# BUTSpeechFIT/DiariZen

Hardware: AMD Instinct MI355X
Metric: audio-seconds/s (RTF) for wavlm-large-s80 pipeline, 16 kHz mono (higher is better)
Workload: dtype f32 (operands split into 2 fp16 terms with exact power-of-two scaling = 22 significant bits, 3 fp16 MFMA products, fp32 accumulate: the error-corrected '3xFP16/3xTF32' scheme; kernels without an fp16 variant use the 3-term bf16 split)

## Files before the change

diarizen_amd/_lib.py:

```python
from __future__ import annotations

import ctypes as C
import os
from pathlib import Path

DZN_MAX_CONV = 8
DZN_MAX_LAYERS = 32
DZN_MAX_HEADS = 16

DZN_PREC_F32 = 0
DZN_PREC_BF16 = 1
DZN_PREC_F32_SPLIT = 2
DZN_PREC_F32_H2 = 3
DZN_PREC_F16 = 4

DZN_ACT_NONE, DZN_ACT_GELU, DZN_ACT_SWISH, DZN_ACT_RELU = 0, 1, 2, 3

DZN_F32, DZN_F64, DZN_I64 = 0, 1, 2

ERRORS = {0: "ok", -1: "invalid argument", -2: "out of memory", -3: "HIP runtime error",
          -4: "bad call order", -5: "missing state_dict key"}


class DznError(RuntimeError):
# ... 15 lines not shown
        ("embed_dim", C.c_int32),
        ("total_heads", C.c_int32),
        ("n_layers", C.c_int32),
        ("layer_norm_first", C.c_int32),
        ("pos_conv_kernel", C.c_int32),
        ("pos_conv_groups", C.c_int32),
        ("num_buckets", C.c_int32),
        ("max_distance", C.c_int32),
        ("use_attention", C.c_int32 * DZN_MAX_LAYERS),
        ("n_heads", C.c_int32 * DZN_MAX_LAYERS),
        ("head_idx", (C.c_int32 * DZN_MAX_HEADS) * DZN_MAX_LAYERS),
        ("use_ffn", C.c_int32 * DZN_MAX_LAYERS),
        ("ffn_dim", C.c_int32 * DZN_MAX_LAYERS),
        ("attention_in", C.c_int32),
        ("ffn_hidden", C.c_int32),
        ("conf_heads", C.c_int32),
        ("conf_layers", C.c_int32),
        ("conf_kernel", C.c_int32),
        ("n_classes", C.c_int32),
        ("max_speakers_per_chunk", C.c_int32),
        ("max_speakers_per_frame", C.c_int32),
        ("has_embedding", C.c_int32),
        ("embed_out_dim", C.c_int32),
        ("num_mel_bins", C.c_int32),
        ("reserved", C.c_int32 * 16),
    ]


class DznGemmDesc(C.Structure):
    _fields_ = [
        ("A", C.c_void_p), ("W", C.c_void_p), ("W16", C.c_void_p), ("C", C.c_void_p),
        ("bias", C.c_void_p), ("R", C.c_void_p), ("WS", C.c_void_p),
        ("a_rowoff", C.c_void_p), ("c_rowoff", C.c_void_p),
        ("M", C.c_int32), ("N", C.c_int32), ("K", C.c_int32),
        ("lda", C.c_int64), ("kc", C.c_int32), ("ldk", C.c_int64), ("ldw", C.c_int32),
        ("ldc", C.c_int64), ("ldws", C.c_int64),
        ("act", C.c_int32), ("alpha", C.c_float), ("post_relu", C.c_int32),
        ("ws_w", C.c_float), ("ws_init", C.c_int32),
        ("nz", C.c_int32), ("zdiv", C.c_int32),
        ("a_z0", C.c_int64), ("a_z1", C.c_int64), ("w_z0", C.c_int64), ("w_z1", C.c_int64),
        ("c_z0", C.c_int64), ("c_z1", C.c_int64), ("b_z0", C.c_int64), ("b_z1", C.c_int64),
        ("precision", C.c_int32),
        ("alg_flops", C.c_double),
        ("W3", C.c_void_p),
        ("a_split3", C.c_int32), ("a_plane", C.c_int64),
        ("ln_stats", C.c_void_p), ("ln_colsum", C.c_void_p),
        ("W2h", C.c_void_p), ("col_scale", C.c_void_p), ("a_amax", C.c_void_p), ("c_amax", C.c_void_p),
        ("amax_unit", C.c_int32),
        ("stat_partial", C.c_void_p), ("stat_final", C.c_void_p), ("stat_C", C.c_int32), ("stat_eps", C.c_float),
        ("z_count", C.c_void_p), ("z_list", C.c_void_p),
        ("Wmx", C.c_void_p), ("col_scale_mx", C.c_void_p),
        ("amax_count", C.c_int32),
        ("kv_planes", C.c_void_p), ("kv_plane_stride", C.c_int64), ("kv_scale", C.c_void_p), ("kv_ld", C.c_int32),
        ("kv_col0", C.c_int32),
        ("A2", C.c_void_p), ("a2_rowoff", C.c_void_p), ("a2_amax", C.c_void_p), ("a2_z0", C.c_int64),
        ("k1", C.c_int32), ("k2", C.c_int32),
    ]


class DznProfEntry(C.Structure):
    _fields_ = [("name", C.c_char * 64), ("launches", C.c_int64), ("ms", C.c_double),
                ("flops", C.c_double), ("bytes", C.c_double)]


def lib_path() -> Path:
    env = os.environ.get("DZN_HIP_LIB")
    if env:
        return Path(env)
    return Path(__file__).resolve().parent / "lib" / "libdzn_hip.so"


_LIB = None


def load() -> C.CDLL:
    global _LIB
    if _LIB is not None:
        return _LIB
    p = lib_path()
    if not p.exists():
        raise DznError(
            f"{p} not found: build the HIP extension first (python -m diarizen_amd.build). "
            "diarizen_amd has no CPU fallback.")
    try:
        import torch
    except Exception:
        pass
    lib = C.CDLL(str(p))
    vp, i32, i64, f32 = C.c_void_p, C.c_int32, C.c_int64, C.c_float

    def sig(name, res, args):
        fn = getattr(lib, name)
        fn.restype = res
        fn.argtypes = args

    sig("dzn_create", i32, [C.POINTER(DznConfig), C.POINTER(vp)])
    sig("dzn_load_tensor", i32, [vp, C.c_char_p, vp, C.POINTER(i64), i32, i32])
    sig("dzn_finalize_weights", i32, [vp])
    sig("dzn_num_frames", i32, [vp, i32])
    sig("dzn_segment_forward", i32, [vp, vp, i32, i32, vp, vp, vp])
    sig("dzn_segment_forward_soft", i32, [vp, vp, i32, i32, vp, vp, vp, vp])
    sig("dzn_embed_forward", i32, [vp, vp, vp, i32, i32, i32, i32, vp, vp])
    sig("dzn_prepare_masks", i32, [vp, vp, i32, i32, i32, i32, i32, vp, vp, vp])
    sig("dzn_speaker_count", i32, [vp, i32, i32, i32, vp, i32, vp, vp, vp])
    sig("dzn_cluster_activations", i32, [vp, vp, i32, i32, i32, vp, i32, i32, vp, vp])
    sig("dzn_detect", i32, [vp, i32, i32, i32, vp, vp, i32, i32, f32, f32, vp, vp, vp])
    sig("dzn_speaker_scores", i32, [vp, vp, i32, i32, i32, vp, vp, vp, i32, i32, vp, vp])
    sig("dzn_debug_fetch", i32, [vp, C.c_char_p, vp, i64, C.POINTER(i64)])
    sig("dzn_embed_skip_stats", i32, [vp, C.POINTER(i64), C.POINTER(i64)])
    sig("dzn_num_ignored", i32, [vp])
    sig("dzn_workspace_bytes", i64, [vp])
    sig("dzn_last_error", C.c_char_p, [vp])
    sig("dzn_destroy", i32, [vp])
    sig("dzn_version", C.c_char_p, [])
    sig("dzn_profile_enable", i32, [i32])
    sig("dzn_profile_collect", i32, [C.POINTER(DznProfEntry), i32, C.POINTER(i32)])
    sig("dzn_profile_reserve", i32, [i32])
    sig("dzn_op_relpos_bucket", i32, [i32, i32, i32])
    sig("dzn_linkage_centroid", i32, [vp, i32, i32, vp, i32])
    sig("dzn_cdist_cosine", i32, [vp, i32, i32, vp, i32, vp, i32])
    sig("dzn_host_workspace_release", i32, [i32])
    sig("dzn_host_workspace_bytes", i64, [i32])
    sig("dzn_vbx_create", i32, [vp, vp, vp, i32, i32, i32, i32, C.POINTER(C.c_void_p)])
    sig("dzn_vbx_stats", i32, [vp, vp])
    sig("dzn_vbx_estep", i32, [vp, vp, vp, vp, C.c_double, C.POINTER(C.c_double)])
    sig("dzn_vbx_gamma", i32, [vp, vp])
    sig("dzn_vbx_destroy", i32, [vp])
    sig("dzn_op_gemm", i32, [C.POINTER(DznGemmDesc), vp])
    sig("dzn_op_split_weights", i32, [vp, i64, i32, i64, vp, vp])
    sig("dzn_op_split_weights_h2", i32, [vp, i64, i32, i64, vp, vp, vp])
    sig("dzn_op_split_weights_mx", i32, [vp, i64, i32, i64, vp, vp, vp])
    sig("dzn_op_set_gemm_mx_cfg", i32, [C.c_char_p])
    sig("dzn_checked_status", i32, [vp, i32])
    sig("dzn_flac_info", i32, [vp, C.c_size_t, vp, vp, vp, vp, vp])
    sig("dzn_flac_decode", i32, [vp, C.c_size_t, vp, i64, vp])
    sig("dzn_op_set_gemm_cfg", i32, [C.c_char_p])
    sig("dzn_op_amax", i32, [vp, i64, vp, vp])
    sig("dzn_op_split_rows", i32, [vp, vp, i64, i64, i32, vp])
    sig("dzn_op_conv3x3_c32", i32, [vp, vp, vp, vp, vp, i32, i32, i32, i32, i32, vp])
    sig("dzn_op_resblock_ws", i32, [vp, vp, vp, vp, vp, vp, vp, vp, vp, f32, f32, i32, i32, i32, i32, vp])
    sig("dzn_op_resblock32_fused", i32, [vp, vp, vp, vp, vp, vp, vp, vp, vp, f32, f32, i32, i32, i32, vp])
    sig("dzn_op_set_resblock_np", i32, [i32])
    sig("dzn_op_set_attention_noskip", i32, [i32])
    sig("dzn_op_conv3x3_c32_h2", i32, [vp, vp, vp, vp, vp, vp, vp, vp, i32, i32, i32, i32, i32, vp])
    sig("dzn_op_layernorm", i32, [vp, i64, vp, i64, vp, vp, i64, i32, i32, f32, i32, vp])
    sig("dzn_op_gate", i32, [vp, i64, vp, vp, vp, vp, i64, i32, vp])
    sig("dzn_op_row_stats", i32, [vp, i64, i64, i32, f32, vp, vp])
    sig("dzn_op_gate_stats", i32, [vp, i64, vp, vp, vp, vp, vp, vp, vp, i64, i32, f32, vp])
    sig("dzn_op_attention_h2", i32, [vp, vp, vp, vp, vp, i32, i32, i32, i32, i32, i32, f32, vp, vp])
    sig("dzn_op_set_attention_qb", i32, [i32])
    sig("dzn_op_set_attention_prefetch", i32, [i32])
    sig("dzn_op_attention_planes", i32, [vp, vp, vp, vp, vp, i32, i32, i32, i32, i32, i32, f32, vp, vp, vp, vp])
    sig("dzn_op_attention", i32, [vp, vp, vp, vp, vp, i32, i32, i32, i32, i32, i32, f32, i32, vp])
    _LIB = lib
    return lib


EXPORTED = [
    "dzn_create", "dzn_load_tensor", "dzn_finalize_weights", "dzn_num_frames",
    "dzn_segment_forward", "dzn_segment_forward_soft", "dzn_embed_forward", "dzn_prepare_masks", "dzn_speaker_count", "dzn_cluster_activations", "dzn_detect", "dzn_speaker_scores", "dzn_debug_fetch", "dzn_embed_skip_stats", "dzn_num_ignored",
    "dzn_workspace_bytes", "dzn_last_error", "dzn_destroy", "dzn_version", "dzn_linkage_centroid", "dzn_cdist_cosine", "dzn_host_workspace_release",
    "dzn_host_workspace_bytes",
    "dzn_flac_info", "dzn_flac_decode", "dzn_vbx_create", "dzn_vbx_stats", "dzn_vbx_estep", "dzn_vbx_gamma", "dzn_vbx_destroy",
    "dzn_op_gemm", "dzn_op_split_weights", "dzn_op_split_weights_h2", "dzn_op_split_weights_mx", "dzn_op_set_gemm_mx_cfg", "dzn_checked_status", "dzn_op_set_gemm_cfg", "dzn_op_amax", "dzn_op_conv3x3_c32", "dzn_op_conv3x3_c32_h2", "dzn_op_resblock32_fused", "dzn_op_resblock_ws", "dzn_op_set_resblock_np", "dzn_op_set_attention_noskip", "dzn_op_split_rows", "dzn_op_layernorm", "dzn_op_row_stats", "dzn_op_gate", "dzn_op_gate_stats", "dzn_op_attention", "dzn_op_attention_h2", "dzn_op_attention_planes", "dzn_op_set_attention_qb", "dzn_op_set_attention_prefetch",
    "dzn_profile_enable", "dzn_profile_collect", "dzn_profile_reserve", "dzn_op_relpos_bucket",
]


def profile_enable(on: bool) -> None:
    check(load().dzn_profile_enable(int(on)), None, "dzn_profile_enable")


def profile_reserve(n_events: int) -> None:
    check(load().dzn_profile_reserve(int(n_events)), None, "dzn_profile_reserve")


def profile_collect() -> list:
    lib = load()
    arr = (DznProfEntry * 512)()
    n = C.c_int32(0)
    check(lib.dzn_profile_collect(arr, 512, C.byref(n)), None, "dzn_profile_collect")
    return [dict(name=arr[i].name.decode(), launches=arr[i].launches, ms=arr[i].ms,
                 flops=arr[i].flops, bytes=arr[i].bytes) for i in range(min(n.value, 512))]


def check(rc: int, handle=None, what: str = "") -> None:
    if rc == 0:
        return
    msg = ERRORS.get(rc, f"error {rc}")
    try:
        detail = load().dzn_last_error(handle)
        if detail:
            msg += ": " + detail.decode(errors="replace")
    except Exception:
        pass
    if rc == -2:
        raise MemoryError(f"{what}: {msg}")
    raise DznError(f"{what}: {msg}")
```

diarizen_amd/csrc/conformer.hip:

```cpp
#include "common.h"

namespace {

constexpr int DW_TT = 32;

template <int KS>
__global__ __launch_bounds__(256) void glu_dwconv_kernel(const float* __restrict__ u, int64_t ldu,
                                                         const float* __restrict__ w,
                                                         const float* __restrict__ bias,
                                                         float* __restrict__ out, int64_t ldo, int L,
                                                         int A) {
  constexpr int PAD = (KS - 1) / 2;
  constexpr int NIN = DW_TT + KS - 1;
  const int b = blockIdx.y;
  const int t0 = blockIdx.x * DW_TT;
  for (int c = threadIdx.x; c < A; c += blockDim.x) {
    float wr[KS];
#pragma unroll
    for (int j = 0; j < KS; ++j) wr[j] = w[c * KS + j];
    const float bc = bias[c];
    float in[NIN];
#pragma unroll
    for (int i = 0; i < NIN; ++i) {
      const int t = t0 - PAD + i;
      float v = 0.f;
      if (t >= 0 && t < L) {
        const float* up = u + ((int64_t)b * L + t) * ldu;
        v = up[c] * sigmoidf_(up[A + c]);
      }
      in[i] = v;
    }
#pragma unroll
    for (int t = 0; t < DW_TT; ++t) {
      if (t0 + t < L) {
        float a = 0.f;
#pragma unroll
        for (int j = 0; j < KS; ++j) a = fmaf(in[t + j], wr[j], a);
        a += bc;
        out[((int64_t)b * L + t0 + t) * ldo + c] = swishf_(a);
      }
    }
  }
}

__global__ __launch_bounds__(256) void classify_kernel(const float* __restrict__ z, int64_t ldz,
                                                       const float* __restrict__ W,
                                                       const float* __restrict__ bias,
                                                       const uint8_t* __restrict__ mapping,
                                                       int64_t rows, int A, int NC, int S,
                                                       float* __restrict__ logp,
                                                       uint8_t* __restrict__ multilabel,
                                                       float* __restrict__ soft) {
  const int lane = threadIdx.x & 63, wave = threadIdx.x >> 6;
  const int64_t row = (int64_t)blockIdx.x * 4 + wave;
  if (row >= rows) return;
  const float* zp = z + row * ldz;
  float logit[16];
#pragma unroll
  for (int c = 0; c < 16; ++c) logit[c] = 0.f;
  for (int i = lane; i < A; i += 64) {
    const float v = zp[i];
#pragma unroll
    for (int c = 0; c < 16; ++c)
      if (c < NC) logit[c] = fmaf(v, W[c * A + i], logit[c]);
  }
  float mx = -INFINITY;
  int arg = 0;
#pragma unroll
  for (int c = 0; c < 16; ++c) {
    if (c < NC) {
      logit[c] = wave_sum(logit[c]) + bias[c];
      if (logit[c] > mx) { mx = logit[c]; arg = c; }
    }
  }
  float se = 0.f;
#pragma unroll
  for (int c = 0; c < 16; ++c)
    if (c < NC) se += expf(logit[c] - mx);
  const float lse = mx + logf(se);
  if (logp) {
#pragma unroll
    for (int c = 0; c < 16; ++c)
      if (c < NC && lane == c) logp[row * NC + c] = logit[c] - lse;
  }
  if (multilabel && lane < S) multilabel[row * S + lane] = mapping[arg * S + lane];
  if (soft && lane < S) {
    float p = 0.f;
#pragma unroll
    for (int c = 0; c < 16; ++c)
      if (c < NC && mapping[c * S + lane]) p += expf(logit[c] - lse);
    soft[row * S + lane] = p;
  }
}

}

int launch_glu_dwconv(const float* u, int64_t ldu, const float* w, const float* bias, float* out,
                      int64_t ldo, int B, int L, int A, int ks, hipStream_t st) {
  ProfScope prof_scope_(st, "glu_dwconv", 0.0, (double)B * L * A * 12.0);
  dim3 grid((L + DW_TT - 1) / DW_TT, B);
  const int threads = A >= 256 ? 256 : (A >= 128 ? 128 : 64);
#define DZN_DW(KSV) \
  hipLaunchKernelGGL((glu_dwconv_kernel<KSV>), grid, dim3(threads), 0, st, u, ldu, w, bias, out, ldo, L, A)
  if (ks == 31) DZN_DW(31);
  else if (ks == 7) DZN_DW(7);
  else if (ks == 15) DZN_DW(15);
  else return DZN_E_INVALID;
#undef DZN_DW
  return hipGetLastError() == hipSuccess ? DZN_OK : DZN_E_HIP;
}

int launch_classify(const float* z, int64_t ldz, const float* W, const float* bias,
                    const uint8_t* mapping, int64_t rows, int A, int NC, int S, float* logp,
                    uint8_t* multilabel, float* soft, hipStream_t st) {
  ProfScope prof_scope_(st, "classify", 2.0 * (double)rows * A * NC,
                        (double)rows * (A * 4.0 + NC * 4.0 + S + (soft ? S * 4.0 : 0.0)));
  if (NC > 16 || S > 64) return DZN_E_INVALID;
  hipLaunchKernelGGL(classify_kernel, dim3((unsigned)cdiv64(rows, 4)), dim3(256), 0, st, z, ldz, W,
                     bias, mapping, rows, A, NC, S, logp, multilabel, soft);
  return hipGetLastError() == hipSuccess ? DZN_OK : DZN_E_HIP;
}
```

diarizen_amd/csrc/embed.hip:

```cpp

#include "common.h"

namespace {

__global__ __launch_bounds__(256) void frame_prep_kernel(const float* __restrict__ wave, int N,
                                                         int T, int flen, int fshift, int Kp,
                                                         const float* __restrict__ window,
                                                         float preemph, float* __restrict__ frames) {
  const int lane = threadIdx.x & 63, wv = threadIdx.x >> 6;
  const int b = blockIdx.y;
  const int t = blockIdx.x * 4 + wv;
  if (t >= T) return;
  const float* xp = wave + (int64_t)b * N + (int64_t)t * fshift;
  float v[8];
  float s = 0.f;
#pragma unroll
  for (int i = 0; i < 8; ++i) {
    const int idx = lane + 64 * i;
    v[i] = idx < flen ? xp[idx] * 32768.0f : 0.f;
    s += v[i];
  }
  const float mean = wave_sum(s) / (float)flen;
  float* op = frames + ((int64_t)b * T + t) * Kp;
  float pv[8];
#pragma unroll
  for (int i = 0; i < 8; ++i) {
    float prev = __shfl_up(v[i], 1, 64);
    const float prev_reg = __shfl(v[i > 0 ? i - 1 : 0], 63, 64);
    if (lane == 0) prev = i > 0 ? prev_reg : v[0];
    pv[i] = prev;
  }
#pragma unroll
  for (int i = 0; i < 8; ++i) {
    const int idx = lane + 64 * i;
    if (idx < flen) {
      const float cur = v[i] - mean;
      const float prev = pv[i] - mean;
      op[idx] = (cur - preemph * prev) * window[idx];
    } else if (idx < Kp) {
      op[idx] = 0.f;
    }
  }
}

__global__ __launch_bounds__(256) void power_kernel(const float* __restrict__ spec, int64_t rows,
                                                    int nb, float* __restrict__ pw) {
  const int64_t n = rows * nb;
  for (int64_t i = (int64_t)blockIdx.x * 256 + threadIdx.x; i < n; i += (int64_t)gridDim.x * 256) {
    const int64_t r = i / nb;
    const int f = (int)(i - r * nb);
    const float re = spec[r * 2 * nb + f], im = spec[r * 2 * nb + nb + f];
    const float a = sqrtf(re * re + im * im);
    pw[i] = a * a;
  }
}

__global__ __launch_bounds__(256) void log_cmn_kernel(float* __restrict__ mel, int T, int NB,
                                                      float eps) {
  __shared__ float red[16][17];
  const int b = blockIdx.y;
  const int bin = blockIdx.x * 16 + (threadIdx.x & 15);
  const int ph = threadIdx.x >> 4;
  float* mp = mel + (int64_t)b * T * NB;
  float s = 0.f;
  if (bin < NB)
    for (int t = ph; t < T; t += 16) {
      const float v = logf(fmaxf(mp[(int64_t)t * NB + bin], eps));
      mp[(int64_t)t * NB + bin] = v;
      s += v;
    }
  red[ph][threadIdx.x & 15] = s;
  __syncthreads();
  float tot = 0.f;
  for (int i = 0; i < 16; ++i) tot += red[i][threadIdx.x & 15];
  const float mean = tot / (float)T;
  if (bin < NB)
    for (int t = ph; t < T; t += 16) mp[(int64_t)t * NB + bin] -= mean;
}

__global__ __launch_bounds__(256) void stem_conv_kernel(const float* __restrict__ fb, int B, int T,
                                                        int NB, int C,
                                                        const float* __restrict__ w,
                                                        const float* __restrict__ bias,
                                                        float* __restrict__ img, float* __restrict__ amax,
                                                        const int* __restrict__ z_count, const int* __restrict__ z_list) {
  const int cq = C >> 2;
  int b = blockIdx.y;
  if (z_list) {
    if (b >= z_count[0]) return;
    b = z_list[b];
  }
  const int q = threadIdx.x % cq, pl = threadIdx.x / cq, ppb = 256 / cq;
  float wr[4][9], br[4];
#pragma unroll
  for (int c = 0; c < 4; ++c) {
    br[c] = bias[q * 4 + c];
#pragma unroll
    for (int k = 0; k < 9; ++k) wr[c][k] = w[(q * 4 + c) * 9 + k];
  }
  const int npix = NB * T;
  const int per = (npix + gridDim.x - 1) / gridDim.x;
  const int p0 = blockIdx.x * per, p1 = min(npix, p0 + per);
  const float* fbb = fb + (int64_t)b * T * NB;
  float* ib = img + (int64_t)b * (NB + 2) * (T + 2) * C;
  float mx = 0.f;
  for (int p = p0 + pl; p < p1; p += ppb) {
    const int h = p / T, wv = p - h * T;
    float in[9];
#pragma unroll
    for (int dh = 0; dh < 3; ++dh)
#pragma unroll
      for (int dw = 0; dw < 3; ++dw) {
        const int hh = h + dh - 1, ww = wv + dw - 1;
        in[dh * 3 + dw] = (hh >= 0 && hh < NB && ww >= 0 && ww < T) ? fbb[(int64_t)ww * NB + hh] : 0.f;
      }
    float o[4];
#pragma unroll
    for (int c = 0; c < 4; ++c) {
      float acc = 0.f;
#pragma unroll
      for (int k = 0; k < 9; ++k) acc = fmaf(in[k], wr[c][k], acc);
      o[c] = fmaxf(acc + br[c], 0.f);
    }
    float* op = ib + ((int64_t)(h + 1) * (T + 2) + wv + 1) * C + q * 4;
    *reinterpret_cast<float4*>(op) = make_float4(o[0], o[1], o[2], o[3]);
    mx = fmaxf(mx, fmaxf(fmaxf(o[0], o[1]), fmaxf(o[2], o[3])));
  }
  if (amax) {
    __shared__ float wmax[4];
    const float m = wave_max(mx);
    if ((threadIdx.x & 63) == 0) wmax[threadIdx.x >> 6] = m;
    __syncthreads();
    if (threadIdx.x == 0) track_amax_lane(amax + b, fmaxf(fmaxf(wmax[0], wmax[1]), fmaxf(wmax[2], wmax[3])));
  }
}

__global__ __launch_bounds__(256) void stats_pool_kernel(const float* __restrict__ img, int H, int W,
                                                         int C, const float* __restrict__ masks,
                                                         int S, int L, float* __restrict__ stats,
                                                         const int* __restrict__ active) {
  extern __shared__ float sw[];
  const int b = blockIdx.y, h = blockIdx.x;
  if (active && !active[b]) {
    for (int c = threadIdx.x; c < C; c += blockDim.x)
      for (int s = 0; s < S; ++s) {
        float* op = stats + ((int64_t)b * S + s) * (2 * C * H);
        op[c * H + h] = 0.f;
        op[C * H + c * H + h] = 0.f;
      }
    return;
  }
  const float scale = (float)L / (float)W;
  for (int i = threadIdx.x; i < S * W; i += blockDim.x) {
    const int s = i / W, t = i - s * W;
    int src = (int)floorf((float)t * scale);
    src = src < L - 1 ? src : L - 1;
    sw[i] = (W == L) ? masks[((int64_t)b * S + s) * L + t] : masks[((int64_t)b * S + s) * L + src];
  }
  __syncthreads();
  const float* base = img + (((int64_t)b * (H + 2) + h + 1) * (W + 2) + 1) * C;
  for (int c = threadIdx.x; c < C; c += blockDim.x) {
    for (int s = 0; s < S; ++s) {
      const float* wt = sw + s * W;
      float v1 = 0.f, v2 = 0.f, sx = 0.f;
      for (int t = 0; t < W; ++t) {
        const float wv = wt[t];
        v1 += wv;
        v2 += wv * wv;
        sx += base[(int64_t)t * C + c] * wv;
      }
      v1 += 1e-8f;
      const float mean = sx / v1;
      float sq = 0.f;
      for (int t = 0; t < W; ++t) {
        const float d = base[(int64_t)t * C + c] - mean;
        sq += d * d * wt[t];
      }
      const float var = sq / (v1 - v2 / v1 + 1e-8f);
      float* op = stats + ((int64_t)b * S + s) * (2 * C * H);
      op[c * H + h] = mean;
      op[C * H + c * H + h] = sqrtf(var);
    }
  }
}

__global__ __launch_bounds__(256) void window_active_kernel(const float* __restrict__ masks, int per_window,
                                                            int* __restrict__ flag) {
  const float* m = masks + (int64_t)blockIdx.x * per_window;
  int any = 0;
  for (int i = threadIdx.x; i < per_window; i += 256) any |= m[i] != 0.f;
  any = __syncthreads_or(any);
  if (threadIdx.x == 0) flag[blockIdx.x] = any != 0;
}

__global__ __launch_bounds__(256) void compact_active_kernel(const int* __restrict__ flag, int B, int* __restrict__ count,
                                                             int* __restrict__ list, long long* __restrict__ totals) {
  __shared__ int wsum[4];
  __shared__ int base;
  const int lane = threadIdx.x & 63, wave = threadIdx.x >> 6;
  if (threadIdx.x == 0) base = 0;
  __syncthreads();
  for (int b0 = 0; b0 < B; b0 += 256) {
    const int b = b0 + threadIdx.x;
    const int f = b < B ? (flag[b] != 0) : 0;
    const unsigned long long bal = __ballot(f);
    const int before = __popcll(bal & ((1ull << lane) - 1ull));
    if (lane == 0) wsum[wave] = __popcll(bal);
    __syncthreads();
    int off = base;
    for (int w = 0; w < wave; ++w) off += wsum[w];
    if (f) list[off + before] = b;
    __syncthreads();
    if (threadIdx.x == 0) base += wsum[0] + wsum[1] + wsum[2] + wsum[3];
    __syncthreads();
  }
  if (threadIdx.x == 0) {
    count[0] = base;
    if (totals) {
      totals[0] += B;
      totals[1] += B - base;
    }
  }
}

inline unsigned grid_for(int64_t n, int per = 256, int cap = 8192) {
  int64_t g = cdiv64(n, per);
  return (unsigned)(g < 1 ? 1 : (g > cap ? cap : g));
}

}

int launch_frame_prep(const float* wave, int B, int N, int T, int flen, int fshift, int Kp,
                      const float* window, float preemph, float* frames, hipStream_t st) {
  ProfScope prof_scope_(st, "frame_prep", 0.0, (double)B * N * 4.0 + (double)B * T * Kp * 4.0);
  if (flen > 512 || T <= 0) return DZN_E_INVALID;
  hipLaunchKernelGGL(frame_prep_kernel, dim3((T + 3) / 4, B), dim3(256), 0, st, wave, N, T, flen,
                     fshift, Kp, window, preemph, frames);
  return hipGetLastError() == hipSuccess ? DZN_OK : DZN_E_HIP;
}

int launch_window_active(const float* masks, int B, int per_window, int* flag, hipStream_t st) {
  ProfScope prof_scope_(st, "window_active", 0.0, (double)B * per_window * 4.0);
  hipLaunchKernelGGL(window_active_kernel, dim3(B), dim3(256), 0, st, masks, per_window, flag);
  return hipGetLastError() == hipSuccess ? DZN_OK : DZN_E_HIP;
}

int launch_compact_active(const int* flag, int B, int* count, int* list, long long* totals, hipStream_t st) {
  hipLaunchKernelGGL(compact_active_kernel, dim3(1), dim3(256), 0, st, flag, B, count, list, totals);
  return hipGetLastError() == hipSuccess ? DZN_OK : DZN_E_HIP;
}

int launch_power(const float* spec, int64_t rows, int nb, float* pw, hipStream_t st) {
  ProfScope prof_scope_(st, "power", 0.0, (double)rows * nb * 12.0);
  hipLaunchKernelGGL(power_kernel, dim3(grid_for(rows * nb)), dim3(256), 0, st, spec, rows, nb, pw);
  return hipGetLastError() == hipSuccess ? DZN_OK : DZN_E_HIP;
}

int launch_log_cmn(float* mel, int B, int T, int NB, float eps, hipStream_t st) {
  ProfScope prof_scope_(st, "log_cmn", 0.0, (double)B * T * NB * 12.0);
  hipLaunchKernelGGL(log_cmn_kernel, dim3((NB + 15) / 16, B), dim3(256), 0, st, mel, T, NB, eps);
  return hipGetLastError() == hipSuccess ? DZN_OK : DZN_E_HIP;
}

int launch_stem_conv(const float* fb, int B, int T, int NB, int C, const float* w, const float* bias,
                     float* img, hipStream_t st, float* amax, const int* z_count, const int* z_list) {
  ProfScope prof_scope_(st, "stem_conv", 2.0 * B * NB * (double)T * C * 9.0,
                        (double)B * NB * T * 4.0 + (double)B * NB * T * C * 4.0);
  if (C % 4 || 256 % (C / 4)) return DZN_E_INVALID;
  const int npix = NB * T, ppb = 256 / (C / 4);
  int gx = (npix + 8 * ppb - 1) / (8 * ppb);
  gx = gx < 1 ? 1 : gx;
  const dim3 grid(gx, B);
  hipLaunchKernelGGL(stem_conv_kernel, grid, dim3(256), 0, st, fb, B, T, NB, C, w, bias, img, amax, z_count, z_list);
  return hipGetLastError() == hipSuccess ? DZN_OK : DZN_E_HIP;
}

int launch_stats_pool(const float* img, int B, int H, int W, int C, const float* masks, int S,
                      int L, float* stats, hipStream_t st, const int* active) {
  ProfScope prof_scope_(st, "stats_pool", 0.0, (double)B * H * W * C * 4.0 + (double)B * S * L * 4.0);
  const size_t lds = (size_t)S * W * sizeof(float);
  hipLaunchKernelGGL(stats_pool_kernel, dim3(H, B), dim3(256), lds, st, img, H, W, C, masks, S, L, stats, active);
  return hipGetLastError() == hipSuccess ? DZN_OK : DZN_E_HIP;
}
```

diarizen_amd/ops.py:

```python
from __future__ import annotations

import ctypes as C

import torch

from . import _lib
from ._lib import DznGemmDesc, check


def _stream() -> C.c_void_p:
    return C.c_void_p(torch.cuda.current_stream().cuda_stream)


def _p(t):
    return None if t is None else C.c_void_p(t.data_ptr())


def gemm(A, W, *, M=None, N=None, K=None, bias=None, R=None, C_out=None, WS=None, ws_w=0.0,
         ws_init=False, a_rowoff=None, c_rowoff=None, lda=None, kc=0, ldk=0, ldw=None, ldc=None,
         ldws=0, act=0, alpha=1.0, post_relu=False, nz=1, zdiv=1, zs=None, precision=0,
         W16=None, W3=None, a_planes=None, ln_stats=None, ln_colsum=None, W2h=None, col_scale=None,
         a_amax=None, c_amax=None, amax_unit=None, want_row_stats=False, stat_eps=1e-5, mx=False, Wmx=None,
         col_scale_mx=None, kv_col0=None, A2=None, a2_rowoff=None, a2_z0=0, k1=0, k2=0, a2_amax=None):
    lib = _lib.load()
# ... 151 lines not shown
    B, Hp, Wp, _ = img.shape
    if out is None:
        out = torch.zeros_like(img)
    am = img.reshape(B, -1).abs().amax(dim=1).float().contiguous()
    (W1, cs1), (W2, cs2) = h2_w1, h2_w2
    check(lib.dzn_op_resblock32_fused(_p(img), _p(out), _p(W1), _p(cs1), _p(b1), _p(W2), _p(cs2), _p(b2), _p(am),
                                      float(l1max1), float(bmax1), B, Hp - 2, Wp - 2, _stream()),
          what="dzn_op_resblock32_fused")
    return out


def resblock_ws(img, h2_w1, b1, h2_w2, b2, l1max1: float, bmax1: float, out=None):
    lib = _lib.load()
    assert img.is_cuda and img.dtype == torch.float32 and img.is_contiguous() and img.shape[-1] in (32, 64)
    B, Hp, Wp, Cn = img.shape
    if out is None:
        out = torch.zeros_like(img)
    am = img.reshape(B, -1).abs().amax(dim=1).float().contiguous()
    (W1, cs1), (W2, cs2) = h2_w1, h2_w2
    check(lib.dzn_op_resblock_ws(_p(img), _p(out), _p(W1), _p(cs1), _p(b1), _p(W2), _p(cs2), _p(b2), _p(am), float(l1max1),
                                 float(bmax1), B, Hp - 2, Wp - 2, Cn, _stream()), what="dzn_op_resblock_ws")
    return out


def linkage_centroid(emb, device: int = -1):
    import numpy as np
    lib = _lib.load()
    e = np.ascontiguousarray(emb, dtype=np.float32)
    n, dim = e.shape
    Z = np.empty((n - 1, 4), dtype=np.float64)
    check(lib.dzn_linkage_centroid(e.ctypes.data_as(C.c_void_p), n, dim, Z.ctypes.data_as(C.c_void_p), device),
          what="dzn_linkage_centroid")
    return Z


def cdist_cosine(emb, centroids, device: int = -1):
    import numpy as np
    lib = _lib.load()
    e = np.ascontiguousarray(emb, dtype=np.float32)
    c = np.ascontiguousarray(centroids, dtype=np.float64)
    n, dim = e.shape
    k = c.shape[0]
    assert c.shape[1] == dim
    out = np.empty((n, k), dtype=np.float64)
    check(lib.dzn_cdist_cosine(e.ctypes.data_as(C.c_void_p), n, dim, c.ctypes.data_as(C.c_void_p), k,
                               out.ctypes.data_as(C.c_void_p), device), what="dzn_cdist_cosine")
    return out


class VbxState:

    def __init__(self, X, Phi, gamma0, device: int = -1):
        import numpy as np
        self.np, self.lib = np, _lib.load()
        X = np.ascontiguousarray(X, dtype=np.float64)
        Phi = np.ascontiguousarray(Phi, dtype=np.float64)
        g0 = np.ascontiguousarray(gamma0, dtype=np.float64)
        self.E, self.D = X.shape
        self.K = g0.shape[1]
        assert Phi.shape == (self.D,) and g0.shape[0] == self.E
        self.state = C.c_void_p()
        check(self.lib.dzn_vbx_create(X.ctypes.data_as(C.c_void_p), Phi.ctypes.data_as(C.c_void_p),
                                      g0.ctypes.data_as(C.c_void_p), self.E, self.D, self.K, device,
                                      C.byref(self.state)), what="dzn_vbx_create")

    def stats(self):
        out = self.np.empty((self.K, self.D + 1), dtype=self.np.float64)
        check(self.lib.dzn_vbx_stats(self.state, out.ctypes.data_as(C.c_void_p)), what="dzn_vbx_stats")
        return out

    def estep(self, alpha, ck, lpi, Fa: float) -> float:
        np = self.np
        alpha = np.ascontiguousarray(alpha, dtype=np.float64)
        ck = np.ascontiguousarray(ck, dtype=np.float64)
        lpi = np.ascontiguousarray(lpi, dtype=np.float64)
        assert alpha.shape == (self.K, self.D) and ck.shape == (self.K,) and lpi.shape == (self.K,)
        total = C.c_double(0.0)
        check(self.lib.dzn_vbx_estep(self.state, alpha.ctypes.data_as(C.c_void_p), ck.ctypes.data_as(C.c_void_p),
                                     lpi.ctypes.data_as(C.c_void_p), float(Fa), C.byref(total)), what="dzn_vbx_estep")
        return total.value

    def gamma(self):
        out = self.np.empty((self.E, self.K), dtype=self.np.float64)
        check(self.lib.dzn_vbx_gamma(self.state, out.ctypes.data_as(C.c_void_p)), what="dzn_vbx_gamma")
        return out

    def close(self):
        if self.state:
            self.lib.dzn_vbx_destroy(self.state)
            self.state = C.c_void_p()

    def __del__(self):
        try:
            self.close()
        except Exception:
            pass


def layernorm(x, gamma, beta, C_true=None, eps=1e-5, gelu=False, out=None):
    lib = _lib.load()
    rows, ld = x.shape[0], x.stride(0)
    Cpad = x.shape[1]
    if C_true is None:
        C_true = Cpad
    if out is None:
        out = torch.empty_like(x)
    check(lib.dzn_op_layernorm(_p(x), ld, _p(out), out.stride(0), _p(gamma), _p(beta), rows,
                               C_true, Cpad, eps, int(gelu), _stream()), what="dzn_op_layernorm")
    return out


def row_stats(x, C_true=None, eps=1e-5):
    lib = _lib.load()
    rows = x.shape[0]
    out = torch.empty((rows, 2), device=x.device, dtype=torch.float32)
    check(lib.dzn_op_row_stats(_p(x), x.stride(0), rows, C_true or x.shape[1], eps, _p(out), _stream()),
          what="dzn_op_row_stats")
    return out


def gate_stats(x, gamma, beta, Wg, bg, cst, eps=1e-5):
    lib = _lib.load()
    rows, Htot = x.shape[0], cst.numel()
    gate_ = torch.empty((rows, Htot), device=x.device, dtype=torch.float32)
    stats = torch.empty((rows, 2), device=x.device, dtype=torch.float32)
    check(lib.dzn_op_gate_stats(_p(x), x.stride(0), _p(gamma), _p(beta), _p(Wg), _p(bg), _p(cst), _p(gate_), _p(stats),
                                rows, Htot, eps, _stream()), what="dzn_op_gate_stats")
    return gate_, stats


def gate(y, Wg, bg, cst):
    lib = _lib.load()
    rows = y.shape[0]
    Htot = cst.numel()
    out = torch.empty((rows, Htot), device=y.device, dtype=torch.float32)
    check(lib.dzn_op_gate(_p(y), y.stride(0), _p(Wg), _p(bg), _p(cst), _p(out), rows, Htot,
                          _stream()), what="dzn_op_gate")
    return out


def attention(qkv, B, L, h, *, gate=None, table=None, head_idx=None, Htot=0, scale=0.125,
              precision=0):
    lib = _lib.load()
    out = torch.empty((B * L, h * 64), device=qkv.device, dtype=torch.float32)
    if precision == _lib.DZN_PREC_F32_H2:
        am = qkv.reshape(B, -1).abs().amax(dim=1).float().contiguous()
        check(lib.dzn_op_attention_h2(_p(qkv), _p(out), _p(gate), _p(table), _p(head_idx), B, L, h, Htot,
                                      qkv.stride(0), out.stride(0), scale, _p(am), _stream()), what="dzn_op_attention_h2")
        return out
    check(lib.dzn_op_attention(_p(qkv), _p(out), _p(gate), _p(table), _p(head_idx), B, L, h,
                               Htot, qkv.stride(0), out.stride(0), scale, precision, _stream()),
          what="dzn_op_attention")
    return out
```

include/dzn_ops.h:

```cpp
#ifndef DZN_OPS_H_
#define DZN_OPS_H_

#include <stdint.h>

#ifdef __cplusplus
extern "C" {
#endif

#define DZN_ACT_NONE 0
#define DZN_ACT_GELU 1
#define DZN_ACT_SWISH 2
#define DZN_ACT_RELU 3

typedef struct dzn_gemm_desc {
  const float* A;
  const float* W;
  const void* W16;
  float* C;
  const float* bias;
  const float* R;
  float* WS;
  const int32_t* a_rowoff;
  const int32_t* c_rowoff;
  int32_t M, N, K;
  int64_t lda;
  int32_t kc;
  int64_t ldk;
  int32_t ldw;
  int64_t ldc;
  int64_t ldws;
  int32_t act;
  float alpha;
  int32_t post_relu;
  float ws_w;
  int32_t ws_init;
  int32_t nz, zdiv;
  int64_t a_z0, a_z1, w_z0, w_z1, c_z0, c_z1, b_z0, b_z1;
  int32_t precision;
  double alg_flops;
  const void* W3;
  int32_t a_split3;
  int64_t a_plane;
  const float* ln_stats;
  const float* ln_colsum;
  const void* W2h;
  const float* col_scale;
  const float* a_amax;
  float* c_amax;
  int32_t amax_unit;
  float* stat_partial;
  float* stat_final;
  int32_t stat_C;
  float stat_eps;
  const int32_t* z_count;
  const int32_t* z_list;
  const void* Wmx;
  const float* col_scale_mx;
  int32_t amax_count;
  void* kv_planes;
  int64_t kv_plane_stride;
  float* kv_scale;
  int32_t kv_ld;
  int32_t kv_col0;
  const float* A2;
  const int32_t* a2_rowoff;
  const float* a2_amax;
  int64_t a2_z0;
  int32_t k1, k2;
} dzn_gemm_desc;

int dzn_op_resblock32_fused(const float* in, float* out, const void* W1, const float* cs1, const float* b1, const void* W2,
                            const float* cs2, const float* b2, const float* amax_in, float l1max1, float bmax1, int32_t B,
                            int32_t Hs, int32_t Ws, void* stream);

int dzn_op_resblock_ws(const float* in, float* out, const void* W1, const float* cs1, const float* b1, const void* W2,
                       const float* cs2, const float* b2, const float* amax_in, float l1max1, float bmax1, int32_t B,
                       int32_t Hs, int32_t Ws, int32_t C, void* stream);

int dzn_op_set_resblock_np(int32_t np);
int dzn_op_set_attention_noskip(int32_t on);

int dzn_op_gemm(const dzn_gemm_desc* d, void* stream);

int dzn_op_split_weights(const float* W, int64_t rows, int32_t K, int64_t ldw, void* W3, void* stream);

int dzn_op_split_weights_h2(const float* W, int64_t rows, int32_t K, int64_t ldw, void* W2h, float* col_scale,
                            void* stream);

int dzn_op_split_weights_mx(const float* W, int64_t rows, int32_t K, int64_t ldw, void* Wmx, float* col_scale,
                            void* stream);
int dzn_checked_status(uint32_t* out4, int32_t reset);

int dzn_op_set_gemm_mx_cfg(const char* cfg);

int dzn_op_set_gemm_cfg(const char* cfg);

int dzn_op_amax(const float* x, int64_t n, float* amax, void* stream);

int dzn_op_split_rows(const float* x, void* planes, int64_t plane_stride, int64_t rows, int32_t D, void* stream);

int dzn_op_conv3x3_c32(const float* in, const void* W3, const float* bias, const float* R, float* out,
                       int32_t B, int32_t Hs, int32_t Ws, int32_t relu, int32_t post_relu, void* stream);

int dzn_op_conv3x3_c32_h2(const float* in, const void* W3, const void* W2h, const float* col_scale, const float* amax_in,
                          const float* bias, const float* R, float* out, int32_t B, int32_t Hs, int32_t Ws,
                          int32_t relu, int32_t post_relu, void* stream);

int dzn_op_layernorm(const float* x, int64_t ldx, float* y, int64_t ldy, const float* gamma,
                     const float* beta, int64_t rows, int32_t C, int32_t Cpad, float eps,
                     int32_t gelu, void* stream);

int dzn_op_row_stats(const float* x, int64_t ldx, int64_t rows, int32_t C, float eps, float* stats, void* stream);

int dzn_op_gate(const float* y, int64_t ldy, const float* Wg, const float* bg, const float* cst,
                float* gate, int64_t rows, int32_t Htot, void* stream);

int dzn_op_gate_stats(const float* x, int64_t ldx, const float* gamma, const float* beta, const float* Wg,
                      const float* bg, const float* cst, float* gate, float* stats, int64_t rows, int32_t Htot,
                      float eps, void* stream);

int dzn_op_attention_h2(const float* qkv, float* out, const float* gate, const float* table, const int32_t* head_idx,
                        int32_t B, int32_t L, int32_t h, int32_t Htot, int32_t ldqkv, int32_t ldo, float scale,
                        const float* amax, void* stream);

int dzn_op_attention_planes(const float* qkv, float* out, const float* gate, const float* table, const int32_t* head_idx,
                            int32_t B, int32_t L, int32_t h, int32_t Htot, int32_t ldqkv, int32_t ldo, float scale,
                            const float* amax, void* planes, float* kvs, void* stream);

int dzn_op_set_attention_qb(int32_t query_blocks_per_wavefront);
int dzn_op_set_attention_prefetch(int32_t on);

int dzn_op_attention(const float* qkv, float* out, const float* gate, const float* table,
                     const int32_t* head_idx, int32_t B, int32_t L, int32_t h,
                     int32_t Htot, int32_t ldqkv, int32_t ldo, float scale,
                     int32_t precision, void* stream);

typedef struct dzn_prof_entry {
  char name[64];
  int64_t launches;
  double ms;
  double flops;
  double bytes;
} dzn_prof_entry;
int dzn_profile_enable(int32_t on);
int dzn_profile_collect(dzn_prof_entry* out, int32_t cap, int32_t* n);
int dzn_profile_reserve(int32_t n_events);

int dzn_op_relpos_bucket(int32_t rel, int32_t num_buckets, int32_t max_distance);

#ifdef __cplusplus
}
#endif
#endif
```

Baseline: 1783.

## Retile GLU depthwise conv, frame prep, and stats pooling kernels with LDS staging

Restructures three small kernels. The GLU+depthwise conv now tiles over time and channel blocks and computes the gated input once into shared memory, instead of each thread recomputing overlapping windows. Frame prep stages a shared waveform span and window for 16 frames per block and can use float4 stores. Stats pooling gives each thread one (h,c) feature and keeps its time series in registers instead of rereading global memory per speaker. It also exposes these kernels as standalone ops, at the cost of more register and LDS pressure.

```diff
diff --git a/diarizen_amd/_lib.py b/diarizen_amd/_lib.py
--- a/diarizen_amd/_lib.py
+++ b/diarizen_amd/_lib.py
@@ -191,6 +191,10 @@
     sig("dzn_op_set_attention_prefetch", i32, [i32])
     sig("dzn_op_attention_planes", i32, [vp, vp, vp, vp, vp, i32, i32, i32, i32, i32, i32, f32, vp, vp, vp, vp])
     sig("dzn_op_attention", i32, [vp, vp, vp, vp, vp, i32, i32, i32, i32, i32, i32, f32, i32, vp])
+    sig("dzn_op_glu_dwconv", i32, [vp, i64, vp, vp, vp, i64, i32, i32, i32, i32, vp])
+    sig("dzn_op_classify", i32, [vp, i64, vp, vp, vp, i64, i32, i32, i32, vp, vp, vp, vp])
+    sig("dzn_op_frame_prep", i32, [vp, i32, i32, i32, i32, i32, i32, vp, f32, vp, vp])
+    sig("dzn_op_stats_pool", i32, [vp, i32, i32, i32, i32, vp, i32, i32, vp, vp, vp])
     _LIB = lib
     return lib
 
@@ -203,6 +207,7 @@
     "dzn_flac_info", "dzn_flac_decode", "dzn_vbx_create", "dzn_vbx_stats", "dzn_vbx_estep", "dzn_vbx_gamma", "dzn_vbx_destroy",
     "dzn_op_gemm", "dzn_op_split_weights", "dzn_op_split_weights_h2", "dzn_op_split_weights_mx", "dzn_op_set_gemm_mx_cfg", "dzn_checked_status", "dzn_op_set_gemm_cfg", "dzn_op_amax", "dzn_op_conv3x3_c32", "dzn_op_conv3x3_c32_h2", "dzn_op_resblock32_fused", "dzn_op_resblock_ws", "dzn_op_set_resblock_np", "dzn_op_set_attention_noskip", "dzn_op_split_rows", "dzn_op_layernorm", "dzn_op_row_stats", "dzn_op_gate", "dzn_op_gate_stats", "dzn_op_attention", "dzn_op_attention_h2", "dzn_op_attention_planes", "dzn_op_set_attention_qb", "dzn_op_set_attention_prefetch",
     "dzn_profile_enable", "dzn_profile_collect", "dzn_profile_reserve", "dzn_op_relpos_bucket",
+    "dzn_op_glu_dwconv", "dzn_op_classify", "dzn_op_frame_prep", "dzn_op_stats_pool",
 ]
 
 
diff --git a/diarizen_amd/csrc/conformer.hip b/diarizen_amd/csrc/conformer.hip
--- a/diarizen_amd/csrc/conformer.hip
+++ b/diarizen_amd/csrc/conformer.hip
@@ -2,43 +2,69 @@
 
 namespace {
 
-constexpr int DW_TT = 32;
+constexpr int DW_TT = 128;
+constexpr int DW_CH = 64;
+constexpr int DW_RUN = 32;
 
-template <int KS>
+template <int KS, bool VEC>
 __global__ __launch_bounds__(256) void glu_dwconv_kernel(const float* __restrict__ u, int64_t ldu,
                                                          const float* __restrict__ w,
                                                          const float* __restrict__ bias,
                                                          float* __restrict__ out, int64_t ldo, int L,
                                                          int A) {
   constexpr int PAD = (KS - 1) / 2;
-  constexpr int NIN = DW_TT + KS - 1;
-  const int b = blockIdx.y;
+  constexpr int NROW = DW_TT + KS - 1;
+  constexpr int NIN = DW_RUN + KS - 1;
+  __shared__ __attribute__((aligned(16))) float g[NROW * DW_CH];
+  const int b = blockIdx.z;
   const int t0 = blockIdx.x * DW_TT;
-  for (int c = threadIdx.x; c < A; c += blockDim.x) {
-    float wr[KS];
-#pragma unroll
-    for (int j = 0; j < KS; ++j) wr[j] = w[c * KS + j];
-    const float bc = bias[c];
-    float in[NIN];
-#pragma unroll
-    for (int i = 0; i < NIN; ++i) {
-      const int t = t0 - PAD + i;
+  const int c0 = blockIdx.y * DW_CH;
+  const float* ub = u + (int64_t)b * L * ldu;
+  if (VEC) {
+    for (int i = threadIdx.x; i < NROW * (DW_CH / 4); i += 256) {
+      const int r = i / (DW_CH / 4), c = c0 + (i % (DW_CH / 4)) * 4;
+      const int t = t0 - PAD + r;
+      float4 v = make_float4(0.f, 0.f, 0.f, 0.f);
+      if (t >= 0 && t < L && c < A) {
+        const float* up = ub + (int64_t)t * ldu;
+        const float4 x = *reinterpret_cast<const float4*>(up + c);
+        const float4 y = *reinterpret_cast<const float4*>(up + A + c);
+        v = make_float4(x.x * sigmoidf_(y.x), x.y * sigmoidf_(y.y), x.z * sigmoidf_(y.z), x.w * sigmoidf_(y.w));
+      }
+      *reinterpret_cast<float4*>(&g[r * DW_CH + (c - c0)]) = v;
+    }
+  } else {
+    for (int i = threadIdx.x; i < NROW * DW_CH; i += 256) {
+      const int r = i / DW_CH, c = c0 + i % DW_CH;
+      const int t = t0 - PAD + r;
       float v = 0.f;
-      if (t >= 0 && t < L) {
-        const float* up = u + ((int64_t)b * L + t) * ldu;
+      if (t >= 0 && t < L && c < A) {
+        const float* up = ub + (int64_t)t * ldu;
         v = up[c] * sigmoidf_(up[A + c]);
       }
-      in[i] = v;
+      g[i] = v;
     }
+  }
+  __syncthreads();
+  const int cl = threadIdx.x % DW_CH, run = threadIdx.x / DW_CH;
+  const int c = c0 + cl;
+  const int tr = t0 + run * DW_RUN;
+  if (c >= A || tr >= L) return;
+  float wr[KS];
 #pragma unroll
-    for (int t = 0; t < DW_TT; ++t) {
-      if (t0 + t < L) {
-        float a = 0.f;
+  for (int j = 0; j < KS; ++j) wr[j] = w[c * KS + j];
+  const float bc = bias[c];
+  float in[NIN];
 #pragma unroll
-        for (int j = 0; j < KS; ++j) a = fmaf(in[t + j], wr[j], a);
-        a += bc;
-        out[((int64_t)b * L + t0 + t) * ldo + c] = swishf_(a);
-      }
+  for (int i = 0; i < NIN; ++i) in[i] = g[(run * DW_RUN + i) * DW_CH + cl];
+#pragma unroll
+  for (int t = 0; t < DW_RUN; ++t) {
+    if (tr + t < L) {
+      float a = 0.f;
+#pragma unroll
+      for (int j = 0; j < KS; ++j) a = fmaf(in[t + j], wr[j], a);
+      a += bc;
+      out[((int64_t)b * L + tr + t) * ldo + c] = swishf_(a);
     }
   }
 }
@@ -98,10 +124,14 @@
 int launch_glu_dwconv(const float* u, int64_t ldu, const float* w, const float* bias, float* out,
                       int64_t ldo, int B, int L, int A, int ks, hipStream_t st) {
   ProfScope prof_scope_(st, "glu_dwconv", 0.0, (double)B * L * A * 12.0);
-  dim3 grid((L + DW_TT - 1) / DW_TT, B);
-  const int threads = A >= 256 ? 256 : (A >= 128 ? 128 : 64);
-#define DZN_DW(KSV) \
-  hipLaunchKernelGGL((glu_dwconv_kernel<KSV>), grid, dim3(threads), 0, st, u, ldu, w, bias, out, ldo, L, A)
+  if (B <= 0 || L <= 0 || A <= 0) return DZN_E_INVALID;
+  dim3 grid((L + DW_TT - 1) / DW_TT, (A + DW_CH - 1) / DW_CH, B);
+  const bool vec = A % 4 == 0 && ldu % 4 == 0 && (reinterpret_cast<uintptr_t>(u) & 15) == 0;
+#define DZN_DW(KSV)                                                                                                    \
+  do {                                                                                                                 \
+    if (vec) hipLaunchKernelGGL((glu_dwconv_kernel<KSV, true>), grid, dim3(256), 0, st, u, ldu, w, bias, out, ldo, L, A); \
+    else hipLaunchKernelGGL((glu_dwconv_kernel<KSV, false>), grid, dim3(256), 0, st, u, ldu, w, bias, out, ldo, L, A);   \
+  } while (0)
   if (ks == 31) DZN_DW(31);
   else if (ks == 7) DZN_DW(7);
   else if (ks == 15) DZN_DW(15);
@@ -120,3 +150,17 @@
                      bias, mapping, rows, A, NC, S, logp, multilabel, soft);
   return hipGetLastError() == hipSuccess ? DZN_OK : DZN_E_HIP;
 }
+
+extern "C" int dzn_op_glu_dwconv(const float* u, int64_t ldu, const float* w, const float* bias, float* out, int64_t ldo,
+                                 int32_t B, int32_t L, int32_t A, int32_t ks, void* stream) {
+  if (!u || !w || !bias || !out || ldu < 2 * (int64_t)A || ldo < A) return DZN_E_INVALID;
+  return launch_glu_dwconv(u, ldu, w, bias, out, ldo, B, L, A, ks, reinterpret_cast<hipStream_t>(stream));
+}
+
+extern "C" int dzn_op_classify(const float* z, int64_t ldz, const float* W, const float* bias, const uint8_t* mapping,
+                               int64_t rows, int32_t A, int32_t NC, int32_t S, float* logp, uint8_t* multilabel,
+                               float* soft, void* stream) {
+  if (!z || !W || !bias || !mapping || A <= 0 || NC <= 0 || S <= 0 || ldz < A) return DZN_E_INVALID;
+  return launch_classify(z, ldz, W, bias, mapping, rows, A, NC, S, logp, multilabel, soft,
+                         reinterpret_cast<hipStream_t>(stream));
+}
diff --git a/diarizen_amd/csrc/embed.hip b/diarizen_amd/csrc/embed.hip
--- a/diarizen_amd/csrc/embed.hip
+++ b/diarizen_amd/csrc/embed.hip
@@ -3,42 +3,61 @@
 
 namespace {
 
+constexpr int FP_FPW = 16;
+
+template <bool VEC>
 __global__ __launch_bounds__(256) void frame_prep_kernel(const float* __restrict__ wave, int N,
                                                          int T, int flen, int fshift, int Kp,
                                                          const float* __restrict__ window,
                                                          float preemph, float* __restrict__ frames) {
+  extern __shared__ __attribute__((aligned(16))) float fp_lds[];
+  float* win = fp_lds;
+  float* x = fp_lds + flen;
   const int lane = threadIdx.x & 63, wv = threadIdx.x >> 6;
   const int b = blockIdx.y;
-  const int t = blockIdx.x * 4 + wv;
-  if (t >= T) return;
-  const float* xp = wave + (int64_t)b * N + (int64_t)t * fshift;
-  float v[8];
-  float s = 0.f;
-#pragma unroll
-  for (int i = 0; i < 8; ++i) {
-    const int idx = lane + 64 * i;
-    v[i] = idx < flen ? xp[idx] * 32768.0f : 0.f;
-    s += v[i];
-  }
-  const float mean = wave_sum(s) / (float)flen;
-  float* op = frames + ((int64_t)b * T + t) * Kp;
-  float pv[8];
-#pragma unroll
-  for (int i = 0; i < 8; ++i) {
-    float prev = __shfl_up(v[i], 1, 64);
-    const float prev_reg = __shfl(v[i > 0 ? i - 1 : 0], 63, 64);
-    if (lane == 0) prev = i > 0 ? prev_reg : v[0];
-    pv[i] = prev;
-  }
-#pragma unroll
-  for (int i = 0; i < 8; ++i) {
-    const int idx = lane + 64 * i;
-    if (idx < flen) {
-      const float cur = v[i] - mean;
-      const float prev = pv[i] - mean;
-      op[idx] = (cur - preemph * prev) * window[idx];
-    } else if (idx < Kp) {
-      op[idx] = 0.f;
+  const int t0 = blockIdx.x * FP_FPW;
+  const int nf = min(FP_FPW, T - t0);
+  const int ns = (nf - 1) * fshift + flen;
+  const float* xp = wave + (int64_t)b * N + (int64_t)t0 * fshift;
+  for (int i = threadIdx.x; i < ns; i += 256) x[i] = xp[i] * 32768.0f;
+  for (int i = threadIdx.x; i < flen; i += 256) win[i] = window[i];
+  __syncthreads();
+  for (int f = wv; f < nf; f += 4) {
+    const float* v = x + f * fshift;
+    float s = 0.f;
+#pragma unroll
+    for (int i = 0; i < 8; ++i) {
+      const int idx = lane + 64 * i;
+      s += idx < flen ? v[idx] : 0.f;
+    }
+    const float mean = wave_sum(s) / (float)flen;
+    float* op = frames + ((int64_t)b * T + t0 + f) * Kp;
+    if (VEC) {
+      for (int q = lane; q < Kp / 4; q += 64) {
+        float o[4];
+#pragma unroll
+        for (int j = 0; j < 4; ++j) {
+          const int idx = 4 * q + j;
+          float r = 0.f;
+          if (idx < flen) {
+            const float cur = v[idx] - mean;
+            const float prev = v[idx > 0 ? idx - 1 : 0] - mean;
+            r = (cur - preemph * prev) * win[idx];
+          }
+          o[j] = r;
+        }
+        *reinterpret_cast<float4*>(op + 4 * q) = make_float4(o[0], o[1], o[2], o[3]);
+      }
+    } else {
+      for (int idx = lane; idx < Kp; idx += 64) {
+        float r = 0.f;
+        if (idx < flen) {
+          const float cur = v[idx] - mean;
+          const float prev = v[idx > 0 ? idx - 1 : 0] - mean;
+          r = (cur - preemph * prev) * win[idx];
+        }
+        op[idx] = r;
+      }
     }
   }
 }
@@ -135,20 +154,32 @@
   }
 }
 
+constexpr int SP_WREG = 100;
+
+template <bool REG>
 __global__ __launch_bounds__(256) void stats_pool_kernel(const float* __restrict__ img, int H, int W,
                                                          int C, const float* __restrict__ masks,
                                                          int S, int L, float* __restrict__ stats,
                                                          const int* __restrict__ active) {
   extern __shared__ float sw[];
-  const int b = blockIdx.y, h = blockIdx.x;
+  const int b = blockIdx.y;
+  const int f = blockIdx.x * 256 + threadIdx.x;
+  const int h = f / C, c = f - h * C;
+  const bool own = f < H * C;
   if (active && !active[b]) {
-    for (int c = threadIdx.x; c < C; c += blockDim.x)
+    if (own)
       for (int s = 0; s < S; ++s) {
         float* op = stats + ((int64_t)b * S + s) * (2 * C * H);
         op[c * H + h] = 0.f;
         op[C * H + c * H + h] = 0.f;
       }
     return;
+  }
+  const float* base = img + (((int64_t)b * (H + 2) + h + 1) * (W + 2) + 1) * C + c;
+  float x[REG ? SP_WREG : 1];
+  if (REG) {
+#pragma unroll
+    for (int t = 0; t < SP_WREG; ++t) x[t] = (own && t < W) ? base[(int64_t)t * C] : 0.f;
   }
   const float scale = (float)L / (float)W;
   for (int i = threadIdx.x; i < S * W; i += blockDim.x) {
@@ -158,29 +189,47 @@
     sw[i] = (W == L) ? masks[((int64_t)b * S + s) * L + t] : masks[((int64_t)b * S + s) * L + src];
   }
   __syncthreads();
-  const float* base = img + (((int64_t)b * (H + 2) + h + 1) * (W + 2) + 1) * C;
-  for (int c = threadIdx.x; c < C; c += blockDim.x) {
-    for (int s = 0; s < S; ++s) {
-      const float* wt = sw + s * W;
-      float v1 = 0.f, v2 = 0.f, sx = 0.f;
+  if (!own) return;
+  for (int s = 0; s < S; ++s) {
+    const float* wt = sw + s * W;
+    float v1 = 0.f, v2 = 0.f, sx = 0.f;
+    if (REG) {
+#pragma unroll
+      for (int t = 0; t < SP_WREG; ++t)
+        if (t < W) {
+          const float wv = wt[t];
+          v1 += wv;
+          v2 += wv * wv;
+          sx += x[t] * wv;
+        }
+    } else {
       for (int t = 0; t < W; ++t) {
         const float wv = wt[t];
         v1 += wv;
         v2 += wv * wv;
-        sx += base[(int64_t)t * C + c] * wv;
-      }
-      v1 += 1e-8f;
-      const float mean = sx / v1;
-      float sq = 0.f;
+        sx += base[(int64_t)t * C] * wv;
+      }
+    }
+    v1 += 1e-8f;
+    const float mean = sx / v1;
+    float sq = 0.f;
+    if (REG) {
+#pragma unroll
+      for (int t = 0; t < SP_WREG; ++t)
+        if (t < W) {
+          const float d = x[t] - mean;
+          sq += d * d * wt[t];
+        }
+    } else {
       for (int t = 0; t < W; ++t) {
-        const float d = base[(int64_t)t * C + c] - mean;
+        const float d = base[(int64_t)t * C] - mean;
         sq += d * d * wt[t];
       }
-      const float var = sq / (v1 - v2 / v1 + 1e-8f);
-      float* op = stats + ((int64_t)b * S + s) * (2 * C * H);
-      op[c * H + h] = mean;
-      op[C * H + c * H + h] = sqrtf(var);
-    }
+    }
+    const float var = sq / (v1 - v2 / v1 + 1e-8f);
+    float* op = stats + ((int64_t)b * S + s) * (2 * C * H);
+    op[c * H + h] = mean;
+    op[C * H + c * H + h] = sqrtf(var);
   }
 }
 
@@ -233,9 +282,17 @@
 int launch_frame_prep(const float* wave, int B, int N, int T, int flen, int fshift, int Kp,
                       const float* window, float preemph, float* frames, hipStream_t st) {
   ProfScope prof_scope_(st, "frame_prep", 0.0, (double)B * N * 4.0 + (double)B * T * Kp * 4.0);
-  if (flen > 512 || T <= 0) return DZN_E_INVALID;
-  hipLaunchKernelGGL(frame_prep_kernel, dim3((T + 3) / 4, B), dim3(256), 0, st, wave, N, T, flen,
-                     fshift, Kp, window, preemph, frames);
+  if (flen > 512 || flen <= 0 || fshift <= 0 || Kp < flen || T <= 0 || B <= 0) return DZN_E_INVALID;
+  if ((int64_t)(T - 1) * fshift + flen > N) return DZN_E_INVALID;
+  const size_t lds = ((size_t)flen + (size_t)(FP_FPW - 1) * fshift + flen) * sizeof(float);
+  if (lds > 64 * 1024) return DZN_E_INVALID;
+  const dim3 grid((T + FP_FPW - 1) / FP_FPW, B);
+  if (Kp % 4 == 0 && (reinterpret_cast<uintptr_t>(frames) & 15) == 0)
+    hipLaunchKernelGGL(frame_prep_kernel<true>, grid, dim3(256), lds, st, wave, N, T, flen, fshift, Kp, window, preemph,
+                       frames);
+  else
+    hipLaunchKernelGGL(frame_prep_kernel<false>, grid, dim3(256), lds, st, wave, N, T, flen, fshift, Kp, window, preemph,
+                       frames);
   return hipGetLastError() == hipSuccess ? DZN_OK : DZN_E_HIP;
 }
 
@@ -278,7 +335,25 @@
 int launch_stats_pool(const float* img, int B, int H, int W, int C, const float* masks, int S,
                       int L, float* stats, hipStream_t st, const int* active) {
   ProfScope prof_scope_(st, "stats_pool", 0.0, (double)B * H * W * C * 4.0 + (double)B * S * L * 4.0);
+  if (B <= 0 || H <= 0 || W <= 0 || C <= 0 || S <= 0 || L <= 0) return DZN_E_INVALID;
   const size_t lds = (size_t)S * W * sizeof(float);
-  hipLaunchKernelGGL(stats_pool_kernel, dim3(H, B), dim3(256), lds, st, img, H, W, C, masks, S, L, stats, active);
-  return hipGetLastError() == hipSuccess ? DZN_OK : DZN_E_HIP;
-}
+  if (lds > 64 * 1024) return DZN_E_INVALID;
+  const dim3 grid((unsigned)cdiv64((int64_t)H * C, 256), B);
+  if (W <= SP_WREG)
+    hipLaunchKernelGGL(stats_pool_kernel<true>, grid, dim3(256), lds, st, img, H, W, C, masks, S, L, stats, active);
+  else
+    hipLaunchKernelGGL(stats_pool_kernel<false>, grid, dim3(256), lds, st, img, H, W, C, masks, S, L, stats, active);
+  return hipGetLastError() == hipSuccess ? DZN_OK : DZN_E_HIP;
+}
+
+extern "C" int dzn_op_frame_prep(const float* wave, int32_t B, int32_t N, int32_t T, int32_t flen, int32_t fshift, int32_t Kp,
+                                 const float* window, float preemph, float* frames, void* stream) {
+  if (!wave || !window || !frames) return DZN_E_INVALID;
+  return launch_frame_prep(wave, B, N, T, flen, fshift, Kp, window, preemph, frames, reinterpret_cast<hipStream_t>(stream));
+}
+
+extern "C" int dzn_op_stats_pool(const float* img, int32_t B, int32_t H, int32_t W, int32_t C, const float* masks, int32_t S,
+                                 int32_t L, float* stats, const int32_t* active, void* stream) {
+  if (!img || !masks || !stats) return DZN_E_INVALID;
+  return launch_stats_pool(img, B, H, W, C, masks, S, L, stats, reinterpret_cast<hipStream_t>(stream), active);
+}
diff --git a/diarizen_amd/ops.py b/diarizen_amd/ops.py
--- a/diarizen_amd/ops.py
+++ b/diarizen_amd/ops.py
@@ -327,3 +327,52 @@
                                Htot, qkv.stride(0), out.stride(0), scale, precision, _stream()),
           what="dzn_op_attention")
     return out
+
+
+def glu_dwconv(u, w, bias, B, L, out=None):
+    lib = _lib.load()
+    A, ks = w.shape
+    assert u.is_cuda and u.dtype == torch.float32 and u.shape[0] == B * L and u.stride(1) == 1 and w.is_contiguous()
+    if out is None:
+        out = torch.empty((B * L, A), device=u.device, dtype=torch.float32)
+    check(lib.dzn_op_glu_dwconv(_p(u), u.stride(0), _p(w), _p(bias), _p(out), out.stride(0), B, L, A, ks, _stream()),
+          what="dzn_op_glu_dwconv")
+    return out
+
+
+def classify(z, W, bias, mapping, want_logp=True, want_soft=True):
+    lib = _lib.load()
+    rows, A = z.shape
+    NC, S = mapping.shape
+    assert z.is_cuda and z.dtype == torch.float32 and z.stride(1) == 1 and W.is_contiguous() and mapping.dtype == torch.uint8
+    logp = torch.empty((rows, NC), device=z.device, dtype=torch.float32) if want_logp else None
+    soft = torch.empty((rows, S), device=z.device, dtype=torch.float32) if want_soft else None
+    ml = torch.empty((rows, S), device=z.device, dtype=torch.uint8)
+    check(lib.dzn_op_classify(_p(z), z.stride(0), _p(W), _p(bias), _p(mapping), rows, A, NC, S, _p(logp), _p(ml), _p(soft),
+                              _stream()), what="dzn_op_classify")
+    return logp, ml, soft
+
+
+def frame_prep(wave, window, flen=400, fshift=160, Kp=416, preemph=0.97, out=None):
+    lib = _lib.load()
+    B, N = wave.shape
+    assert wave.is_cuda and wave.dtype == torch.float32 and wave.is_contiguous() and window.numel() == flen
+    T = 1 + (N - flen) // fshift
+    if out is None:
+        out = torch.empty((B * T, Kp), device=wave.device, dtype=torch.float32)
+    assert out.shape == (B * T, Kp) and out.is_contiguous()
+    check(lib.dzn_op_frame_prep(_p(wave), B, N, T, flen, fshift, Kp, _p(window), preemph, _p(out), _stream()),
+          what="dzn_op_frame_prep")
+    return out
+
+
+def stats_pool(img, masks, active=None):
+    lib = _lib.load()
+    B, Hp, Wp, Cn = img.shape
+    S, L = masks.shape[1], masks.shape[2]
+    assert img.is_cuda and img.dtype == torch.float32 and img.is_contiguous() and masks.is_contiguous()
+    assert active is None or active.dtype == torch.int32
+    out = torch.empty((B, S, 2 * Cn * (Hp - 2)), device=img.device, dtype=torch.float32)
+    check(lib.dzn_op_stats_pool(_p(img), B, Hp - 2, Wp - 2, Cn, _p(masks), S, L, _p(out), _p(active), _stream()),
+          what="dzn_op_stats_pool")
+    return out
diff --git a/include/dzn_ops.h b/include/dzn_ops.h
--- a/include/dzn_ops.h
+++ b/include/dzn_ops.h
@@ -135,6 +135,18 @@
                      int32_t Htot, int32_t ldqkv, int32_t ldo, float scale,
                      int32_t precision, void* stream);
 
+int dzn_op_glu_dwconv(const float* u, int64_t ldu, const float* w, const float* bias, float* out, int64_t ldo, int32_t B,
+                      int32_t L, int32_t A, int32_t ks, void* stream);
+
+int dzn_op_classify(const float* z, int64_t ldz, const float* W, const float* bias, const uint8_t* mapping, int64_t rows,
+                    int32_t A, int32_t NC, int32_t S, float* logp, uint8_t* multilabel, float* soft, void* stream);
+
+int dzn_op_frame_prep(const float* wave, int32_t B, int32_t N, int32_t T, int32_t flen, int32_t fshift, int32_t Kp,
+                      const float* window, float preemph, float* frames, void* stream);
+
+int dzn_op_stats_pool(const float* img, int32_t B, int32_t H, int32_t W, int32_t C, const float* masks, int32_t S, int32_t L,
+                      float* stats, const int32_t* active, void* stream);
+
 typedef struct dzn_prof_entry {
   char name[64];
   int64_t launches;
```

Result: no change. 1794 (median of 6 runs) (+0.6%).
